# damien911224/ZeroShotVideoClassification

Measured on AMD Instinct MI355X. Metric: clips/sec (fwd+bwd+step) R(2+1)D-18 16x112x112 bs=22/GPU, higher is better.
Workload: dtype f32; 1 GPU; r2plus1d_18 training step (zero_grad+fwd+MSE+bwd+Adam), 22 clips/GPU 3x16x112x112, random-init, fp32 (BASELINE.json configs[1]); clips_per_gpu=22, global_batch=22, optimizer=Adam lr=1e-3 (torch.optim.Adam), parallelism=dp1, world_size=1, launcher=single process, input=resident

## Files before the change

### include/zsv_hip.h

```cpp
#ifndef ZSV_HIP_H
#define ZSV_HIP_H

#include <stddef.h>
#include <stdint.h>

#ifdef __cplusplus
extern "C" {
#endif

#define ZSV_OK 0
#define ZSV_E_BAD_SHAPE 1
#define ZSV_E_NULL 2
#define ZSV_E_WORKSPACE 3
#define ZSV_E_TOO_LARGE 4
#define ZSV_E_LAUNCH 5
#define ZSV_E_UNSUPPORTED 6

typedef struct zsv_conv_desc {
    int32_t N, Cin, Ti, Hi, Wi;
    int32_t Cout, To, Ho, Wo;
    int32_t kT, kH, kW;
    int32_t sT, sH, sW;
    int32_t pT, pH, pW;
} zsv_conv_desc;
// ... 21 lines not shown
                     void* workspace, size_t workspace_bytes, void* stream);
int32_t zsv_conv3d_dgrad_add_supported(const zsv_conv_desc* d);
int zsv_conv3d_dgrad_add(const zsv_conv_desc* d, const float* dy, const float* w, const float* add, float* dx,
                         void* workspace, size_t workspace_bytes, void* stream);
int32_t zsv_conv3d_dgrad_add_strided_supported(const zsv_conv_desc* d, int32_t st, int32_t sh, int32_t sw);
int zsv_conv3d_dgrad_add_strided(const zsv_conv_desc* d, const float* dy, const float* w, const float* sub, int32_t st, int32_t sh,
                                 int32_t sw, float* dx, void* workspace, size_t workspace_bytes, void* stream);
size_t zsv_conv3d_wgrad_workspace_bytes(const zsv_conv_desc* d);
int zsv_conv3d_wgrad(const zsv_conv_desc* d, const float* x, const float* dy, float* dw,
                     void* workspace, size_t workspace_bytes, void* stream);
size_t zsv_conv3d_wgrad_mask_bytes(const zsv_conv_desc* d);
int zsv_conv3d_wgrad_mask(const zsv_conv_desc* d, void* mask, void* stream);
int zsv_conv3d_wgrad_masked(const zsv_conv_desc* d, const float* x, const float* dy, float* dw, void* workspace,
                            size_t workspace_bytes, const void* mask, void* stream);

int zsv_bn_fwd_train_coeffs(const float* x, int32_t N, int32_t C, int32_t S, const float* gamma, const float* beta,
                            float* save_mean, float* save_invstd, float* running_mean, float* running_var, float momentum,
                            float eps, const float* conv_partials, int32_t stat_tiles, float* coef, int32_t coef_pitch,
                            void* workspace, size_t workspace_bytes, void* stream);
int32_t zsv_conv3d_pre_supported(const zsv_conv_desc* d);
int zsv_conv3d_fwd_pre(const zsv_conv_desc* d, const float* x, const float* pre_coef, int32_t coef_pitch, const float* w,
                       float* y, float* bn_partials, int32_t stat_tiles, void* workspace, size_t workspace_bytes,
                       void* stream);
int zsv_conv3d_wgrad_pre(const zsv_conv_desc* d, const float* x, const float* pre_coef, int32_t coef_pitch,
                         const float* dy, float* dw, void* workspace, size_t workspace_bytes, void* stream);
size_t zsv_channel_sum_workspace_bytes(int32_t N, int32_t C, int32_t S);
int zsv_channel_sum(const float* dy, int32_t N, int32_t C, int32_t S, float* db,
                    void* workspace, size_t workspace_bytes, void* stream);

size_t zsv_bn_workspace_bytes(int32_t N, int32_t C, int32_t S);
int zsv_bn_fwd_train(const float* x, int32_t N, int32_t C, int32_t S, const float* gamma,
                     const float* beta, const float* residual, int fuse_relu, float* y,
                     float* save_mean, float* save_invstd, float* running_mean,
                     float* running_var, float momentum, float eps, void* workspace,
                     size_t workspace_bytes, void* stream);
int zsv_bn_fwd_train_stats(const float* x, int32_t N, int32_t C, int32_t S, const float* gamma,
                           const float* beta, const float* residual, int fuse_relu, float* y,
                           float* save_mean, float* save_invstd, float* running_mean,
                           float* running_var, float momentum, float eps, const float* conv_partials,
                           int32_t stat_tiles, void* workspace, size_t workspace_bytes, void* stream);
int zsv_bn_fwd_eval(const float* x, int32_t N, int32_t C, int32_t S, const float* gamma,
                    const float* beta, const float* running_mean, const float* running_var,
                    const float* residual, int fuse_relu, float eps, float* y, void* workspace,
                    size_t workspace_bytes, void* stream);
int zsv_bn_bwd(const float* dy, const float* x, const float* y, int32_t N, int32_t C, int32_t S,
               const float* gamma, const float* beta, const float* save_mean, const float* save_invstd,
               int fuse_relu, float* dx, float* d_residual, float* dgamma, float* dbeta,
               void* workspace, size_t workspace_bytes, void* stream);
int zsv_bn_bwd_eval(const float* dy, const float* x, const float* y, int32_t N, int32_t C, int32_t S,
                    const float* gamma, const float* beta, const float* running_mean, const float* running_var, float eps,
                    int fuse_relu, float* dx, float* d_residual, float* dgamma, float* dbeta,
                    void* workspace, size_t workspace_bytes, void* stream);
int zsv_bn_eval_coeffs(int32_t C, const float* gamma, const float* beta, const float* running_mean, const float* running_var,
                       float eps, float* coef, int32_t coef_pitch, void* stream);

int zsv_relu_fwd(const float* x, float* y, int64_t n, void* stream);
int zsv_relu_bwd(const float* dy, const float* y, float* dx, int64_t n, void* stream);
int zsv_relu_bwd_bias(const float* dy, const float* y, float* dx, int32_t N, int32_t C, int32_t S, float* db,
                      void* workspace, size_t workspace_bytes, void* stream);
int zsv_add_relu_fwd(const float* a, const float* b, float* y, int64_t n, void* stream);

int zsv_meanpool_fwd(const float* x, int32_t N, int32_t C, int32_t S, float* y, void* stream);
int zsv_meanpool_bwd(const float* dy, int32_t N, int32_t C, int32_t S, float* dx, void* stream);
int zsv_maxpool3d_fwd(const float* x, int32_t N, int32_t C, int32_t Ti, int32_t Hi, int32_t Wi,
                      int32_t kT, int32_t kH, int32_t kW, int32_t pT, int32_t pH, int32_t pW,
                      int32_t To, int32_t Ho, int32_t Wo, float* y, int32_t* argmax, void* stream);
int zsv_maxpool3d_bwd(const float* dy, const int32_t* argmax, int32_t N, int32_t C, int32_t Ti,
                      int32_t Hi, int32_t Wi, int32_t kT, int32_t kH, int32_t kW, int32_t pT,
                      int32_t pH, int32_t pW, int32_t To, int32_t Ho, int32_t Wo, float* dx,
                      void* stream);

size_t zsv_linear_fwd_workspace_bytes(int32_t rows, int32_t in_features, int32_t out_features);
int zsv_linear_fwd(const float* x, const float* w, const float* bias, float* y, int32_t rows,
                   int32_t in_features, int32_t out_features, int fuse_relu, void* workspace,
                   size_t workspace_bytes, void* stream);
size_t zsv_linear_dgrad_workspace_bytes(int32_t rows, int32_t in_features, int32_t out_features);
int zsv_linear_dgrad(const float* dy, const float* w, float* dx, int32_t rows, int32_t in_features,
                     int32_t out_features, void* workspace, size_t workspace_bytes, void* stream);
size_t zsv_linear_wgrad_workspace_bytes(int32_t rows, int32_t in_features, int32_t out_features);
int zsv_linear_wgrad(const float* x, const float* dy, float* dw, int32_t rows,
                     int32_t in_features, int32_t out_features, void* workspace,
                     size_t workspace_bytes, void* stream);

size_t zsv_cosine_topk_workspace_bytes(int32_t rows, int32_t n_classes);
int zsv_cosine_topk(const float* embed, const float* class_embed, int32_t rows, int32_t dim, int32_t n_classes,
                    int32_t k, int32_t* out_index, double* out_dist, void* workspace, size_t workspace_bytes,
                    void* stream);

size_t zsv_split_accuracy_workspace_bytes(int32_t rows, int32_t n_classes);
int zsv_split_accuracy(const float* pred, const float* true_embed, const int64_t* labels, const float* class_embed,
                       int32_t rows, int32_t dim, int32_t n_classes, const int32_t* split_pos, int32_t n_tables,
                       int32_t* counts, int32_t* class_counts, void* workspace, size_t workspace_bytes, void* stream);

int zsv_adam_step(float* p, const float* g, float* exp_avg, float* exp_avg_sq, int64_t n,
                  float lr, float beta1, float beta2, float eps, int32_t step, void* stream);

int32_t zsv_bf16_channel_pitch(int32_t channels);
size_t zsv_conv3d_bf16_blob_bytes(const zsv_conv_desc* d);
int zsv_conv3d_bf16_pack(const zsv_conv_desc* d, const float* w, const float* scale, const float* shift,
                         void* blob, void* stream);
int zsv_conv3d_bf16_pack_dgrad(const zsv_conv_desc* d, const float* w_fwd, void* blob, void* stream);
int zsv_conv3d_bf16_fwd(const zsv_conv_desc* d, const void* x, const void* blob, const void* residual,
                        int fuse_relu, void* y, void* stream);
int32_t zsv_conv3d_bf16_stat_rows(const zsv_conv_desc* d);
int zsv_conv3d_bf16_fwd_stats(const zsv_conv_desc* d, const void* x, const void* blob, void* y, float* bn_partials,
                              int32_t rows_capacity, int32_t* rows, void* stream);
int zsv_clip_to_bf16(const float* x, int32_t N, int32_t C, int32_t T, int32_t H, int32_t W, int32_t padH,
                     int32_t padW, int32_t Hp, int32_t Wp, void* out, void* stream);
int zsv_maxpool3d_bf16(const void* x, int32_t N, int32_t C, int32_t Ti, int32_t Hi, int32_t Wi, int32_t kT, int32_t kH, int32_t kW,
                       int32_t pT, int32_t pH, int32_t pW, int32_t To, int32_t Ho, int32_t Wo, void* y, void* stream);
int zsv_meanpool_bf16(const void* x, int32_t N, int32_t S, int32_t C, float* out, void* stream);

int32_t zsv_fp8_channel_pitch(int32_t channels);
size_t zsv_conv3d_fp8_blob_bytes(const zsv_conv_desc* d);
int zsv_conv3d_fp8_pack(const zsv_conv_desc* d, const float* w, const float* scale, const float* shift, void* blob, void* stream);
int zsv_conv3d_fp8_fwd(const zsv_conv_desc* d, const void* x, const void* blob, const void* residual, int fuse_relu, void* y,
                       void* stream);
int zsv_meanpool_fp8(const void* x, int32_t N, int32_t S, int32_t C, float* out, void* stream);
int zsv_maxpool3d_fp8(const void* x, int32_t N, int32_t C, int32_t Ti, int32_t Hi, int32_t Wi, int32_t kT, int32_t kH, int32_t kW,
                      int32_t pT, int32_t pH, int32_t pW, int32_t To, int32_t Ho, int32_t Wo, void* y, void* stream);
int zsv_absmax_bf16(const void* x, int64_t count, float* amax, void* stream);

size_t zsv_bn_cl_workspace_bytes(int64_t R, int32_t C);
int zsv_bn_cl_fwd_train(const void* z, const void* residual, int64_t R, int32_t C, const float* gamma, const float* beta,
                        float* running_mean, float* running_var, float momentum, float eps, int fuse_relu, void* y,
                        float* save_mean, float* save_invstd, float* save_coef, void* workspace, size_t workspace_bytes, void* stream);
int zsv_bn_cl_fwd_train_stats(const void* z, const void* residual, int64_t R, int32_t C, const float* gamma, const float* beta,
                              float* running_mean, float* running_var, float momentum, float eps, int fuse_relu, void* y,
                              float* save_mean, float* save_invstd, float* save_coef, const float* conv_partials, int32_t conv_rows,
                              void* workspace, size_t workspace_bytes, void* stream);
int zsv_bn_cl_bwd(const void* dy, const void* y, const void* z, int64_t R, int32_t C, const float* gamma, const float* save_mean,
                  const float* save_invstd, const float* fwd_coef, int relu_mask, void* dz, void* g_out, float* dgamma, float* dbeta,
                  void* workspace, size_t workspace_bytes, void* stream);
int zsv_bn_cl_fwd_eval(const void* z, const void* residual, int64_t R, int32_t C, const float* gamma, const float* beta,
                       const float* running_mean, const float* running_var, float eps, int fuse_relu, void* y, float* coef,
                       void* stream);
int zsv_bn_cl_bwd_eval(const void* dy, const void* y, const void* z, int64_t R, int32_t C, const float* coef, int relu_mask, void* dz,
                       void* g_out, float* dgamma, float* dbeta, void* workspace, size_t workspace_bytes, void* stream);
size_t zsv_conv3d_bf16_wgrad_workspace_bytes(const zsv_conv_desc* d);
int zsv_conv3d_bf16_wgrad(const zsv_conv_desc* d, const void* x, const void* dz, float* dw, void* workspace, size_t workspace_bytes,
                          void* stream);
int zsv_maxpool3d_bf16_bwd(const void* dy, const void* x, int32_t N, int32_t C, int32_t Ti, int32_t Hi, int32_t Wi, int32_t kT, int32_t kH,
                           int32_t kW, int32_t pT, int32_t pH, int32_t pW, int32_t To, int32_t Ho, int32_t Wo, void* dx, void* stream);
int zsv_relu_bias_bwd_cl(const void* dy, const void* y, int64_t R, int32_t C, void* g_out, float* dbias, void* workspace,
                         size_t workspace_bytes, void* stream);
int zsv_cl_bf16_to_ncs_f32(const void* x, int32_t N, int32_t S, int32_t C, float* out, void* stream);
int zsv_ncs_f32_to_cl_bf16(const float* x, int32_t N, int32_t S, int32_t C, void* out, void* stream);
int zsv_meanpool_bf16_bwd(const float* dpooled, int32_t N, int32_t S, int32_t C, void* dx, void* stream);

int zsv_clip_transform(const uint8_t* frames_u8, int32_t N, int32_t T, int32_t Hin, int32_t Win,
                       int32_t Hres, int32_t Wres, float inv_scale, int32_t crop,
                       const int32_t* crop_flip_params_device, float* out, void* stream);
#define ZSV_CLIP_ROW 8
int zsv_clip_transform_batch(const int64_t* video_table_device, int32_t B, int32_t n_clips, int32_t T,
                             int32_t crop, float* out, void* stream);

int zsv_still_image_clips(const int64_t* image_table_device, const int32_t* frame_table_device, int32_t B,
                          int32_t n_clips, int32_t T, int32_t crop, int32_t max_side, float* out, void* stream);
int zsv_resample_coeffs(int32_t side, int32_t crop, int32_t* coeffs, int32_t* bounds, void* stream);

typedef struct zsv_adam_tensor {
    float* p;
    const float* g;
    float* exp_avg;
    float* exp_avg_sq;
    int64_t n;
// ... 114 lines not shown
```

### zeroshotvideoclassification_amd/_lib.py

```python
from __future__ import annotations

import ctypes
import os
import threading
from ctypes import POINTER, Structure, c_char_p, c_double, c_float, c_int, c_int32, c_int64, c_size_t, c_void_p

_HERE = os.path.dirname(os.path.abspath(__file__))
LIB_PATH = os.environ.get("ZSV_LIB_PATH") or os.path.join(_HERE, "libzsv_hip.so")


class ConvDesc(Structure):
    _fields_ = [(n, c_int32) for n in (
        "N", "Cin", "Ti", "Hi", "Wi", "Cout", "To", "Ho", "Wo",
        "kT", "kH", "kW", "sT", "sH", "sW", "pT", "pH", "pW")]


_P = c_void_p
SIGNATURES = {
    "zsv_status_string": (c_char_p, [c_int]),
    "zsv_version": (c_char_p, []),
    "zsv_reload_knobs": (c_int32, []),
    "zsv_conv3d_fwd_workspace_bytes": (c_size_t, [POINTER(ConvDesc)]),
    "zsv_conv3d_fwd": (c_int, [POINTER(ConvDesc), _P, _P, _P, _P, c_int, _P, c_size_t, _P]),
    "zsv_conv3d_fwd_stat_tiles": (c_int32, [POINTER(ConvDesc), _P]),
    "zsv_conv3d_fwd_stats": (c_int, [POINTER(ConvDesc), _P, _P, _P, _P, c_int, _P, c_int32, _P, c_size_t, _P]),
    "zsv_conv3d_fwd_add_supported": (c_int32, [POINTER(ConvDesc)]),
    "zsv_conv3d_fwd_add": (c_int, [POINTER(ConvDesc), _P, _P, _P, _P, _P, c_int, _P, c_size_t, _P]),
    "zsv_conv3d_fwd_full": (c_int, [POINTER(ConvDesc), _P, _P, _P, _P, _P, c_int, _P, c_int32, _P, c_size_t, _P]),
    "zsv_conv3d_dgrad_workspace_bytes": (c_size_t, [POINTER(ConvDesc)]),
    "zsv_conv3d_dgrad": (c_int, [POINTER(ConvDesc), _P, _P, _P, _P, c_size_t, _P]),
    "zsv_conv3d_dgrad_add_supported": (c_int32, [POINTER(ConvDesc)]),
    "zsv_conv3d_dgrad_add": (c_int, [POINTER(ConvDesc), _P, _P, _P, _P, _P, c_size_t, _P]),
    "zsv_conv3d_dgrad_add_strided_supported": (c_int32, [POINTER(ConvDesc), c_int32, c_int32, c_int32]),
    "zsv_conv3d_dgrad_add_strided": (c_int, [POINTER(ConvDesc), _P, _P, _P, c_int32, c_int32, c_int32, _P, _P, c_size_t, _P]),
    "zsv_conv3d_wgrad_workspace_bytes": (c_size_t, [POINTER(ConvDesc)]),
    "zsv_conv3d_wgrad": (c_int, [POINTER(ConvDesc), _P, _P, _P, _P, c_size_t, _P]),
    "zsv_conv3d_wgrad_mask_bytes": (c_size_t, [POINTER(ConvDesc)]),
    "zsv_conv3d_wgrad_mask": (c_int, [POINTER(ConvDesc), _P, _P]),
    "zsv_conv3d_wgrad_masked": (c_int, [POINTER(ConvDesc), _P, _P, _P, _P, c_size_t, _P, _P]),
    "zsv_bn_fwd_train_coeffs": (c_int, [_P, c_int32, c_int32, c_int32, _P, _P, _P, _P, _P, _P, c_float, c_float, _P, c_int32, _P,
                                        c_int32, _P, c_size_t, _P]),
    "zsv_conv3d_pre_supported": (c_int32, [POINTER(ConvDesc)]),
    "zsv_conv3d_fwd_pre": (c_int, [POINTER(ConvDesc), _P, _P, c_int32, _P, _P, _P, c_int32, _P, c_size_t, _P]),
    "zsv_conv3d_wgrad_pre": (c_int, [POINTER(ConvDesc), _P, _P, c_int32, _P, _P, _P, c_size_t, _P]),
    "zsv_channel_sum_workspace_bytes": (c_size_t, [c_int32, c_int32, c_int32]),
    "zsv_channel_sum": (c_int, [_P, c_int32, c_int32, c_int32, _P, _P, c_size_t, _P]),
    "zsv_bn_workspace_bytes": (c_size_t, [c_int32, c_int32, c_int32]),
    "zsv_bn_fwd_train": (c_int, [_P, c_int32, c_int32, c_int32, _P, _P, _P, c_int, _P, _P, _P, _P, _P,
                                 c_float, c_float, _P, c_size_t, _P]),
    "zsv_bn_fwd_train_stats": (c_int, [_P, c_int32, c_int32, c_int32, _P, _P, _P, c_int, _P, _P, _P, _P, _P,
                                       c_float, c_float, _P, c_int32, _P, c_size_t, _P]),
    "zsv_bn_fwd_eval": (c_int, [_P, c_int32, c_int32, c_int32, _P, _P, _P, _P, _P, c_int, c_float, _P, _P,
                                c_size_t, _P]),
    "zsv_bn_bwd": (c_int, [_P, _P, _P, c_int32, c_int32, c_int32, _P, _P, _P, _P, c_int, _P, _P, _P, _P, _P,
                           c_size_t, _P]),
    "zsv_bn_bwd_eval": (c_int, [_P, _P, _P, c_int32, c_int32, c_int32, _P, _P, _P, _P, c_float, c_int, _P, _P, _P, _P, _P,
                                c_size_t, _P]),
    "zsv_bn_eval_coeffs": (c_int, [c_int32, _P, _P, _P, _P, c_float, _P, c_int32, _P]),
    "zsv_relu_fwd": (c_int, [_P, _P, c_int64, _P]),
    "zsv_relu_bwd": (c_int, [_P, _P, _P, c_int64, _P]),
    "zsv_relu_bwd_bias": (c_int, [_P, _P, _P, c_int32, c_int32, c_int32, _P, _P, c_size_t, _P]),
    "zsv_add_relu_fwd": (c_int, [_P, _P, _P, c_int64, _P]),
    "zsv_meanpool_fwd": (c_int, [_P, c_int32, c_int32, c_int32, _P, _P]),
    "zsv_meanpool_bwd": (c_int, [_P, c_int32, c_int32, c_int32, _P, _P]),
    "zsv_maxpool3d_fwd": (c_int, [_P] + [c_int32] * 14 + [_P, _P, _P]),
    "zsv_maxpool3d_bwd": (c_int, [_P, _P] + [c_int32] * 14 + [_P, _P]),
    "zsv_linear_fwd_workspace_bytes": (c_size_t, [c_int32, c_int32, c_int32]),
    "zsv_linear_fwd": (c_int, [_P, _P, _P, _P, c_int32, c_int32, c_int32, c_int, _P, c_size_t, _P]),
    "zsv_linear_dgrad_workspace_bytes": (c_size_t, [c_int32, c_int32, c_int32]),
    "zsv_linear_dgrad": (c_int, [_P, _P, _P, c_int32, c_int32, c_int32, _P, c_size_t, _P]),
    "zsv_linear_wgrad_workspace_bytes": (c_size_t, [c_int32, c_int32, c_int32]),
    "zsv_linear_wgrad": (c_int, [_P, _P, _P, c_int32, c_int32, c_int32, _P, c_size_t, _P]),
    "zsv_bf16_channel_pitch": (c_int32, [c_int32]),
    "zsv_conv3d_bf16_blob_bytes": (c_size_t, [POINTER(ConvDesc)]),
    "zsv_conv3d_bf16_pack": (c_int, [POINTER(ConvDesc), _P, _P, _P, _P, _P]),
    "zsv_conv3d_bf16_pack_dgrad": (c_int, [POINTER(ConvDesc), _P, _P, _P]),
    "zsv_conv3d_bf16_fwd": (c_int, [POINTER(ConvDesc), _P, _P, _P, c_int, _P, _P]),
    "zsv_clip_to_bf16": (c_int, [_P] + [c_int32] * 9 + [_P, _P]),
    "zsv_maxpool3d_bf16": (c_int, [_P] + [c_int32] * 14 + [_P, _P]),
    "zsv_meanpool_bf16": (c_int, [_P, c_int32, c_int32, c_int32, _P, _P]),
    "zsv_fp8_channel_pitch": (c_int32, [c_int32]),
    "zsv_conv3d_fp8_blob_bytes": (c_size_t, [POINTER(ConvDesc)]),
    "zsv_conv3d_fp8_pack": (c_int, [POINTER(ConvDesc), _P, _P, _P, _P, _P]),
    "zsv_conv3d_fp8_fwd": (c_int, [POINTER(ConvDesc), _P, _P, _P, c_int, _P, _P]),
    "zsv_meanpool_fp8": (c_int, [_P, c_int32, c_int32, c_int32, _P, _P]),
    "zsv_maxpool3d_fp8": (c_int, [_P] + [c_int32] * 14 + [_P, _P]),
    "zsv_absmax_bf16": (c_int, [_P, c_int64, _P, _P]),
    "zsv_bn_cl_workspace_bytes": (c_size_t, [c_int64, c_int32]),
    "zsv_bn_cl_fwd_train": (c_int, [_P, _P, c_int64, c_int32, _P, _P, _P, _P, c_float, c_float, c_int, _P, _P, _P, _P, _P, c_size_t, _P]),
    "zsv_bn_cl_fwd_train_stats": (c_int, [_P, _P, c_int64, c_int32, _P, _P, _P, _P, c_float, c_float, c_int, _P, _P, _P, _P, _P, c_int32, _P,
                                          c_size_t, _P]),
    "zsv_conv3d_bf16_stat_rows": (c_int32, [POINTER(ConvDesc)]),
    "zsv_conv3d_bf16_fwd_stats": (c_int, [POINTER(ConvDesc), _P, _P, _P, _P, c_int32, _P, _P]),
    "zsv_bn_cl_bwd": (c_int, [_P, _P, _P, c_int64, c_int32, _P, _P, _P, _P, c_int, _P, _P, _P, _P, _P, c_size_t, _P]),
    "zsv_bn_cl_fwd_eval": (c_int, [_P, _P, c_int64, c_int32, _P, _P, _P, _P, c_float, c_int, _P, _P, _P]),
    "zsv_bn_cl_bwd_eval": (c_int, [_P, _P, _P, c_int64, c_int32, _P, c_int, _P, _P, _P, _P, _P, c_size_t, _P]),
    "zsv_conv3d_bf16_wgrad_workspace_bytes": (c_size_t, [POINTER(ConvDesc)]),
    "zsv_conv3d_bf16_wgrad": (c_int, [POINTER(ConvDesc), _P, _P, _P, _P, c_size_t, _P]),
    "zsv_maxpool3d_bf16_bwd": (c_int, [_P, _P] + [c_int32] * 14 + [_P, _P]),
    "zsv_relu_bias_bwd_cl": (c_int, [_P, _P, c_int64, c_int32, _P, _P, _P, c_size_t, _P]),
    "zsv_cl_bf16_to_ncs_f32": (c_int, [_P, c_int32, c_int32, c_int32, _P, _P]),
    "zsv_ncs_f32_to_cl_bf16": (c_int, [_P, c_int32, c_int32, c_int32, _P, _P]),
    "zsv_meanpool_bf16_bwd": (c_int, [_P, c_int32, c_int32, c_int32, _P, _P]),
    "zsv_clip_transform": (c_int, [_P, c_int32, c_int32, c_int32, c_int32, c_int32, c_int32, c_float, c_int32, _P, _P, _P]),
    "zsv_clip_transform_batch": (c_int, [_P, c_int32, c_int32, c_int32, c_int32, _P, _P]),
    "zsv_still_image_clips": (c_int, [_P, _P, c_int32, c_int32, c_int32, c_int32, c_int32, _P, _P]),
    "zsv_resample_coeffs": (c_int, [c_int32, c_int32, _P, _P, _P]),
    "zsv_cosine_topk_workspace_bytes": (c_size_t, [c_int32, c_int32]),
    "zsv_cosine_topk": (c_int, [_P, _P, c_int32, c_int32, c_int32, c_int32, _P, _P, _P, c_size_t, _P]),
    "zsv_split_accuracy_workspace_bytes": (c_size_t, [c_int32, c_int32]),
    "zsv_split_accuracy": (c_int, [_P, _P, _P, _P, c_int32, c_int32, c_int32, _P, c_int32, _P, _P, _P, c_size_t, _P]),
    "zsv_adam_multi": (c_int, [_P, c_int32, c_int64, c_float, c_float, c_float, c_float, c_int32, _P]),
    "zsv_grad_check_multi": (c_int, [_P, c_int32, c_int64, _P, _P]),
    "zsv_adam_multi_scaled": (c_int, [_P, c_int32, c_int64, c_float, c_float, c_float, c_float, _P, _P]),
    "zsv_scaler_update": (c_int, [_P, c_float, c_float, c_int32, _P]),
    "zsv_grad_norm_workspace_bytes": (c_size_t, [c_int64]),
    "zsv_grad_norm_multi": (c_int, [_P, c_int32, c_int64, c_int64, _P, c_size_t, _P, _P]),
    "zsv_grad_norm_finalize": (c_int, [_P, c_int64, c_float, _P, _P, _P]),
    "zsv_grad_unscale_multi": (c_int, [_P, c_int32, c_int64, _P, _P]),
    "zsv_adamw_multi": (c_int, [_P, c_int32, c_int64, c_double, c_float, c_float, c_float, c_double, c_int32, _P, c_int32, _P]),
    "zsv_adamw_multi_scaled": (c_int, [_P, c_int32, c_int64, c_double, c_float, c_float, c_float, c_double, c_int32, _P, _P,
                                       c_int32, _P]),
    "zsv_grad_accum_multi": (c_int, [_P, c_int32, c_int64, c_float, c_int32, _P]),
    "zsv_sgd_multi": (c_int, [_P, c_int32, c_int64, c_double, c_float, c_float, c_int32, c_double, c_int32, _P, _P, c_int32, c_int32,
                              _P, _P, c_float, _P]),
    "zsv_adam_multi_avg": (c_int, [_P, c_int32, c_int64, c_float, c_float, c_float, c_float, c_int32, _P, _P, c_float, _P]),
    "zsv_adam_multi_scaled_avg": (c_int, [_P, c_int32, c_int64, c_float, c_float, c_float, c_float, _P, _P, _P, c_float, _P]),
    "zsv_adamw_multi_avg": (c_int, [_P, c_int32, c_int64, c_double, c_float, c_float, c_float, c_double, c_int32, _P, c_int32,
                                    _P, _P, c_float, _P]),
    "zsv_adamw_multi_scaled_avg": (c_int, [_P, c_int32, c_int64, c_double, c_float, c_float, c_float, c_double, c_int32, _P, _P,
                                           c_int32, _P, _P, c_float, _P]),
    "zsv_avg_multi": (c_int, [_P, c_int32, c_int64, _P, c_float, _P, _P]),
    "zsv_avg_advance": (c_int, [_P, _P, _P]),
    "zsv_swap_multi": (c_int, [_P, c_int32, c_int64, _P]),
    "zsv_adam_step": (c_int, [_P, _P, _P, _P, c_int64, c_float, c_float, c_float, c_float, c_int32, _P]),
    "zsv_conv3d_panel_query": (c_int, [POINTER(ConvDesc), c_int32, c_int32, POINTER(c_size_t)]),
    "zsv_conv3d_panel_job": (c_int, [POINTER(ConvDesc), c_int32, c_int32, _P, _P, c_size_t, _P]),
    "zsv_pack_multi": (c_int, [_P, c_int32, c_int64, _P]),
    "zsv_conv3d_fwd_full_panel": (c_int, [POINTER(ConvDesc), _P, _P, _P, _P, _P, c_int, _P, c_int32, _P, c_size_t, _P, _P, c_size_t]),
    "zsv_conv3d_fwd_pre_panel": (c_int, [POINTER(ConvDesc), _P, _P, c_int32, _P, _P, _P, c_int32, _P, c_size_t, _P, _P, c_size_t]),
    "zsv_conv3d_dgrad_add_panel": (c_int, [POINTER(ConvDesc), _P, _P, _P, _P, _P, c_size_t, _P, _P, c_size_t]),
    "zsv_conv3d_dgrad_add_strided_panel": (c_int, [POINTER(ConvDesc), _P, _P, _P, c_int32, c_int32, c_int32, _P, _P, c_size_t, _P, _P,
                                                   c_size_t]),
}


class PackJob(Structure):
    _fields_ = [("kind", c_int32), ("reserved", c_int32), ("total", c_int64), ("first_block", c_int64), ("w", c_void_p),
                ("out", c_void_p), ("l", c_int64 * 2), ("i", c_int32 * 20)]

_lock = threading.Lock()
# ... 86 lines not shown
```

### zeroshotvideoclassification_amd/csrc/knobs.h

```cpp
#pragma once

#define ZSV_KNOB_LIST(X) \
    X(NO_FUSED_STATS) \
    X(NO_BN_FUSION) \
    X(BF16_NO_SAME) \
    X(BF16_NO_TSAME) \
    X(BF16_NO_SAME64) \
    X(BF16_NO_SAME9) \
    X(BF16_SAME9_MIN_CHUNKS) \
    X(WINOT_NO_T32) \
    X(BF16_GROUP_OUTER) \
    X(BF16_NO_WGRAD) \
    X(BF16_NO_WGRAD_GATHER) \
    X(BF16_WGRAD_WGS) \
    X(NO_DGRAD_S2) \
    X(NO_DGRAD_S2T) \
    X(DGRAD_S2_BN) \
    X(DGRAD_S2_KS) \
    X(NO_DOWN_FUSION) \
    X(DGRAD_S2_NO_X4) \
    X(CONV_CFG) \
    X(NO_SPLITK) \
    X(TAP_KS) \
    X(SPLITK_THRESH) \
    X(NO_CFG5) \
    X(NO_TAP) \
    X(NO_LDS_EPILOGUE) \
    X(WGRAD_CFG) \
    X(WGRAD_BN) \
    X(WGRAD_WGS) \
    X(WGRAD_NO_TWOTAP) \
    X(NO_WGRAD_DMA) \
    X(WGRAD_DMA_TM) \
    X(WGRAD_DMA_TN) \
    X(WGRAD_DMA_SLICES) \
    X(WGRAD_LINEAR_WALK) \
    X(NO_STEM_WGRAD) \
    X(STEM_WGRAD_WGS) \
    X(WGRAD_TRING_RESIDENT) \
    X(WGRAD_TRING_SLICES) \
    X(NO_WGRAD_TRING) \
    X(NO_WGRAD_TWINO) \
    X(WGRAD_WINO_SLICES) \
    X(NO_WINO) \
    X(NO_WGRAD_WINO) \
    X(NO_WGRAD_WINO4) \
    X(WINO_MIN_TILES) \
    X(WINO_NO_SPLITK) \
    X(NO_WINOT) \
    X(WINOT_MIN_TILES) \
    X(BN_NT_MB) \
    X(BN_NO_MASKED_G) \
    X(WINOT_MAX_WASTE) \
    X(NO_WINO_FWD) \
    X(WINO_NO_F43) \
    X(WINOT_NO_F43) \
    X(WINO_NO_X4) \
    X(NO_SLAB_SUM_ROWS) \
    X(SPLITK_REDUCE_SCALAR) \
    X(NO_PACK_TILED) \
    X(NO_T2_DENSE) \
    X(WINO_NO_VW) \
    X(WINO_VW_MIN_WGS) \
    X(WINOT_GENERIC_EPILOGUE) \
    X(WINO_GENERIC_EPILOGUE)

namespace zsv {
enum KnobId {
#define ZSV_KNOB_ENUM(name) K_##name,
    ZSV_KNOB_LIST(ZSV_KNOB_ENUM)
#undef ZSV_KNOB_ENUM
    K_COUNT
};
extern const char* volatile g_knobs[K_COUNT];
}

#define ZSV_KNOB(name) (::zsv::g_knobs[::zsv::K_##name])
```

### zeroshotvideoclassification_amd/network.py

```python
from __future__ import annotations

import torch
import torch.nn.functional as F
from torch import nn

from . import ops
from . import resnet as models
from .layers import Conv3d, Linear, MaxPool3d, ReLU


def get_network(opt):
    name = opt.network
    if "r3d" in name:
        factory = models.r3d_18
    elif "2plus1d" in name:
        factory = models.r2plus1d_18
    elif "c3d" in name:
        return C3D(fixconvs=opt.fixconvs, nopretrained=opt.nopretrained)
    else:
        raise Exception("Network {} not available!".format(name))
    return Model(factory, fixconvs=opt.fixconvs, nopretrained=opt.nopretrained)


def _freeze(module: nn.Module) -> None:
    for p in module.parameters():
        p.requires_grad = False


class MLP(nn.Module):

    def __init__(self, input_dim, hidden_dim, output_dim, num_layers, last_activate=False):
        super().__init__()
        self.num_layers = num_layers
        self.last_activate = last_activate
        widths = [input_dim] + [hidden_dim] * (num_layers - 1) + [output_dim]
        self.layers = nn.ModuleList(Linear(a, b) for a, b in zip(widths[:-1], widths[1:]))

    def forward(self, x):
        last = self.num_layers - 1
        for i, layer in enumerate(self.layers):
            x = layer(x, relu=(i < last))
        return x


class Model(nn.Module):

    def __init__(self, network, fixconvs=False, nopretrained=False):
        super().__init__()
        self.model = network(pretrained=nopretrained)
        if fixconvs:
            _freeze(self.model)
        self.d_model = 256
        self.num_sentences = 1
        self.t_pos_embeds = nn.Embedding(self.num_sentences, 512)
        self.special_tokens = nn.Embedding(1, self.d_model)
        self.feature2input_proj = nn.Linear(512, self.d_model)
        self.encoder = nn.TransformerEncoder(
            nn.TransformerEncoderLayer(d_model=self.d_model, dim_feedforward=self.d_model * 4, nhead=8, dropout=0.1,
                                       activation="gelu"),
            num_layers=6, enable_nested_tensor=False)
        self.output2emb_proj = MLP(512, 512, 300, 2)
        self.reset_parameters()

    def reset_parameters(self):
        nn.init.normal_(self.t_pos_embeds.weight)
        nn.init.xavier_uniform_(self.special_tokens.weight)

    def forward(self, x):
        bs, nc, ch, t, h, w = x.shape
        from . import amp
        if amp.is_autocast_enabled() and x.is_cuda:
            from . import resnet
            if isinstance(self.model, resnet.VideoResNet):
                if self.training:
                    pooled = amp.trunk_features(self.model, x.reshape(bs * nc, ch, t, h, w))
                    return F.normalize(self.output2emb_proj(pooled)), None
                if not torch.is_grad_enabled():
                    from .inference import engine_for
                    return engine_for(self, torch.bfloat16)(x)
        _, feats = self.model(x.reshape(bs * nc, ch, t, h, w))
        pooled = ops.mean_pool(feats)
        emb = F.normalize(self.output2emb_proj(pooled))
        return emb, None


class ResNet18(nn.Module):

    def __init__(self, network, fixconvs=False, nopretrained=True):
        super().__init__()
        self.model = network(pretrained=nopretrained)
        if fixconvs:
            _freeze(self.model)
        self.regressor = Linear(self.model.fc.in_features, 300)
        self.dropout = nn.Dropout(p=0.05)

    def forward(self, x):
        bs, nc, ch, t, h, w = x.shape
        pooled, _ = self.model(x.reshape(bs * nc, ch, t, h, w))
        pooled = pooled.reshape(bs, nc, -1).mean(1)
        return F.normalize(self.regressor(self.dropout(pooled)))


class C3D(nn.Module):

    def __init__(self, fixconvs=False, nopretrained=True):
        super().__init__()
        three = (3, 3, 3)
        one = (1, 1, 1)
        self.conv1 = Conv3d(3, 64, kernel_size=three, padding=one)
        self.pool1 = MaxPool3d(kernel_size=(1, 2, 2), stride=(1, 2, 2))
        self.conv2 = Conv3d(64, 128, kernel_size=three, padding=one)
        self.pool2 = MaxPool3d(kernel_size=(2, 2, 2), stride=(2, 2, 2))
        self.conv3a = Conv3d(128, 256, kernel_size=three, padding=one)
        self.conv3b = Conv3d(256, 256, kernel_size=three, padding=one)
        self.pool3 = MaxPool3d(kernel_size=(2, 2, 2), stride=(2, 2, 2))
        self.conv4a = Conv3d(256, 512, kernel_size=three, padding=one)
        self.conv4b = Conv3d(512, 512, kernel_size=three, padding=one)
        self.pool4 = MaxPool3d(kernel_size=(2, 2, 2), stride=(2, 2, 2))
        self.conv5a = Conv3d(512, 512, kernel_size=three, padding=one)
        self.conv5b = Conv3d(512, 512, kernel_size=three, padding=one)
        self.pool5 = MaxPool3d(kernel_size=(2, 2, 2), stride=(2, 2, 2), padding=(0, 1, 1))
        self.fc6 = Linear(8192, 4096)
        self.fc7 = Linear(4096, 4096)
        self.fc8 = Linear(4096, 487)
        self.dropout = nn.Dropout(p=0.10)
        self.relu = ReLU()
        self.softmax = nn.Softmax()
        if nopretrained:
            self.load_state_dict(torch.load("./assets/c3d.pickle"))
        self.regressor = Linear(4096, 300)
        if fixconvs:
            for m in (self.conv1, self.conv2, self.conv3a, self.conv3b, self.conv4a, self.conv4b, self.conv5a,
                      self.conv5b, self.fc6):
                _freeze(m)

    def forward(self, x):
        bs, nc, ch, t, h, w = x.shape
        from . import amp
        if amp.is_autocast_enabled() and x.is_cuda:
            if not torch.is_grad_enabled() and not self.training:
                from .inference import engine_for
                return engine_for(self, torch.bfloat16)(x)
            if torch.is_grad_enabled():
                a = amp.c3d_features(self, x.reshape(bs * nc, ch, t, h, w))
                a = self.fc6(a, relu=True)
                a = self.dropout(a)
                a = a.reshape(bs, nc, -1).mean(1).reshape(bs, -1)
                return F.normalize(self.regressor(a), dim=-1)
        a = x.reshape(bs * nc, ch, t, h, w)
        a = self.pool1(self.conv1(a, relu=True))
        a = self.pool2(self.conv2(a, relu=True))
        a = self.pool3(self.conv3b(self.conv3a(a, relu=True), relu=True))
        a = self.pool4(self.conv4b(self.conv4a(a, relu=True), relu=True))
        a = self.pool5(self.conv5b(self.conv5a(a, relu=True), relu=True))
        a = self.fc6(a.reshape(-1, 8192), relu=True)
        a = self.dropout(a)
        a = a.reshape(bs, nc, -1).mean(1).reshape(bs, -1)
        return F.normalize(self.regressor(a), dim=-1)
```

### zeroshotvideoclassification_amd/ops.py

```python
from __future__ import annotations

import os
import threading

from ctypes import byref, c_size_t, c_void_p
from typing import Optional, Sequence, Tuple

import torch
from torch.autograd import Function
from torch.autograd.function import once_differentiable

from . import _lib
from ._lib import ConvDesc


def _triple(v) -> Tuple[int, int, int]:
    if isinstance(v, int):
        return (v, v, v)
    v = tuple(int(a) for a in v)
    if len(v) == 1:
        return (v[0],) * 3
    if len(v) != 3:
        raise ValueError(f"expected an int or 3 ints, got {v}")
    return v
# ... 998 lines not shown
        dx = torch.empty(geom[:5], dtype=torch.float32, device=dy.device)
        with torch.cuda.device(dy.device):
            _lib.check(_lib.load().zsv_maxpool3d_bwd(dy.data_ptr(), arg.data_ptr(), *geom, dx.data_ptr(), _stream()),
                       "zsv_maxpool3d_bwd")
        return dx, None, None


def max_pool3d(x, kernel_size, stride=None, padding=0):
    k = _triple(kernel_size)
    s = k if stride is None else _triple(stride)
    if s != k:
        raise RuntimeError("max_pool3d: only kernel_size == stride is implemented (all the reference uses)")
    return _MaxPool3d.apply(x, k, _triple(padding))


class _Linear(Function):

    @staticmethod
    def forward(ctx, x, weight, bias, relu):
        _require(x, weight, bias)
        if x.dim() != 2:
            raise RuntimeError("linear expects a (rows, in_features) input")
        x, weight = x.contiguous(), weight.contiguous()
        rows, fin = int(x.shape[0]), int(x.shape[1])
        fout = int(weight.shape[0])
        if int(weight.shape[1]) != fin:
            raise RuntimeError("linear: in_features mismatch")
        y = torch.empty((rows, fout), dtype=torch.float32, device=x.device)
        lib = _lib.load()
        nbytes = lib.zsv_linear_fwd_workspace_bytes(rows, fin, fout)
        ws = _workspace(nbytes, x.device)
        with torch.cuda.device(x.device):
            _lib.check(lib.zsv_linear_fwd(x.data_ptr(), weight.data_ptr(), _ptr(bias), y.data_ptr(), rows, fin,
                                          fout, 1 if relu else 0, _ptr(ws), nbytes, _stream()), "zsv_linear_fwd")
        ctx.dims = (rows, fin, fout)
        ctx.relu = bool(relu)
        ctx.has_bias = bias is not None
        ctx.save_for_backward(x, weight, y if relu else None)
        return y

    @staticmethod
    @once_differentiable
    def backward(ctx, dy):
        x, weight, y = ctx.saved_tensors
        rows, fin, fout = ctx.dims
        lib = _lib.load()
        dy = dy.contiguous()
        dx = dw = db = None
        with torch.cuda.device(dy.device):
            if ctx.relu:
                g = torch.empty_like(dy)
                if ctx.has_bias and ctx.needs_input_grad[2]:
                    n_, c_ = int(dy.shape[0]), int(dy.shape[1])
                    s_ = dy.numel() // (n_ * c_)
                    db = torch.empty(c_, dtype=torch.float32, device=dy.device)
                    nb = lib.zsv_channel_sum_workspace_bytes(n_, c_, s_)
                    wsb = _workspace(nb, dy.device)
                    _lib.check(lib.zsv_relu_bwd_bias(dy.data_ptr(), y.data_ptr(), g.data_ptr(), n_, c_, s_, db.data_ptr(),
                                                     _ptr(wsb), nb, _stream()), "zsv_relu_bwd_bias")
                else:
                    _lib.check(lib.zsv_relu_bwd(dy.data_ptr(), y.data_ptr(), g.data_ptr(), g.numel(), _stream()), "zsv_relu_bwd")
                dy = g
            if ctx.needs_input_grad[0]:
                dx = torch.empty_like(x)
                nbytes = lib.zsv_linear_dgrad_workspace_bytes(rows, fin, fout)
                ws = _workspace(nbytes, dy.device)
                _lib.check(lib.zsv_linear_dgrad(dy.data_ptr(), weight.data_ptr(), dx.data_ptr(), rows, fin, fout,
                                                _ptr(ws), nbytes, _stream()), "zsv_linear_dgrad")
            if ctx.needs_input_grad[1]:
                dw = torch.empty_like(weight)
                nbytes = lib.zsv_linear_wgrad_workspace_bytes(rows, fin, fout)
                ws = _workspace(nbytes, dy.device)
                _lib.check(lib.zsv_linear_wgrad(x.data_ptr(), dy.data_ptr(), dw.data_ptr(), rows, fin, fout, _ptr(ws),
                                                nbytes, _stream()), "zsv_linear_wgrad")
            if ctx.has_bias and ctx.needs_input_grad[2] and db is None:
                db = channel_sum(dy)
        return dx, dw, db, None


def linear(x, weight, bias=None, relu=False):
    return _Linear.apply(x, weight, bias, bool(relu))


def adam_step_(p: torch.Tensor, g: torch.Tensor, exp_avg: torch.Tensor, exp_avg_sq: torch.Tensor, step: int,
               lr: float, betas=(0.9, 0.999), eps: float = 1e-8) -> None:
    _require(p, g, exp_avg, exp_avg_sq)
    for t in (p, g, exp_avg, exp_avg_sq):
        if not t.is_contiguous() or t.numel() != p.numel():
            raise RuntimeError("adam_step_: flat contiguous buffers of equal size expected")
    with torch.cuda.device(p.device):
        _lib.check(_lib.load().zsv_adam_step(p.data_ptr(), g.data_ptr(), exp_avg.data_ptr(), exp_avg_sq.data_ptr(),
                                             p.numel(), float(lr), float(betas[0]), float(betas[1]), float(eps),
                                             int(step), _stream()), "zsv_adam_step")
```

Baseline: 578.8 clips/s.

## Fuse mean-pool, two-layer MLP head and L2 normalize into single HIP kernels

Adds a fused forward kernel that does spatial mean pooling, Linear+ReLU, Linear and L2 normalization per row in one block. A matching fused backward kernel computes the input gradient and all weight and bias gradients. This replaces several small launches (mean pool, linear, normalize and their backward ops) in the model head, cutting launch overhead and intermediate traffic. The kernels accumulate in fp64 and each handles a whole row per block, so they may run slower than tuned GEMMs if the head dimensions are large.

```diff
diff --git a/include/zsv_hip.h b/include/zsv_hip.h
--- a/include/zsv_hip.h
+++ b/include/zsv_hip.h
@@ -127,6 +127,14 @@
                      int32_t in_features, int32_t out_features, void* workspace,
                      size_t workspace_bytes, void* stream);
 
+int32_t zsv_head_supported(int32_t R, int32_t C, int32_t S, int32_t H, int32_t O);
+int zsv_head_fwd(const float* feats, int32_t R, int32_t C, int32_t S, const float* w1, const float* b1, int32_t H,
+                 const float* w2, const float* b2, int32_t O, float eps, float* e, float* p, float* h, float* norm,
+                 void* stream);
+int zsv_head_bwd(const float* de, const float* e, const float* p, const float* h, const float* norm, const float* w1,
+                 const float* w2, int32_t R, int32_t C, int32_t S, int32_t H, int32_t O, float eps, float* dfeats,
+                 float* dw1, float* db1, float* dw2, float* db2, void* stream);
+
 size_t zsv_cosine_topk_workspace_bytes(int32_t rows, int32_t n_classes);
 int zsv_cosine_topk(const float* embed, const float* class_embed, int32_t rows, int32_t dim, int32_t n_classes,
                     int32_t k, int32_t* out_index, double* out_dist, void* workspace, size_t workspace_bytes,
diff --git a/zeroshotvideoclassification_amd/_lib.py b/zeroshotvideoclassification_amd/_lib.py
--- a/zeroshotvideoclassification_amd/_lib.py
+++ b/zeroshotvideoclassification_amd/_lib.py
@@ -67,6 +67,9 @@
     "zsv_maxpool3d_bwd": (c_int, [_P, _P] + [c_int32] * 14 + [_P, _P]),
     "zsv_linear_fwd_workspace_bytes": (c_size_t, [c_int32, c_int32, c_int32]),
     "zsv_linear_fwd": (c_int, [_P, _P, _P, _P, c_int32, c_int32, c_int32, c_int, _P, c_size_t, _P]),
+    "zsv_head_supported": (c_int32, [c_int32] * 5),
+    "zsv_head_fwd": (c_int, [_P, c_int32, c_int32, c_int32, _P, _P, c_int32, _P, _P, c_int32, c_float, _P, _P, _P, _P, _P]),
+    "zsv_head_bwd": (c_int, [_P] * 7 + [c_int32] * 5 + [c_float] + [_P] * 6),
     "zsv_linear_dgrad_workspace_bytes": (c_size_t, [c_int32, c_int32, c_int32]),
     "zsv_linear_dgrad": (c_int, [_P, _P, _P, c_int32, c_int32, c_int32, _P, c_size_t, _P]),
     "zsv_linear_wgrad_workspace_bytes": (c_size_t, [c_int32, c_int32, c_int32]),
diff --git a/zeroshotvideoclassification_amd/csrc/head.hip b/zeroshotvideoclassification_amd/csrc/head.hip
--- /dev/null
+++ b/zeroshotvideoclassification_amd/csrc/head.hip
@@ -0,0 +1,298 @@
+#include <hip/hip_runtime.h>
+#include <stdint.h>
+#include "zsv_hip.h"
+#include "zsv_common.h"
+#include "knobs.h"
+
+namespace zsv {
+
+constexpr int HEAD_THREADS = 1024;
+constexpr int HEAD_WAVES = HEAD_THREADS / 64;
+constexpr int HEAD_JB = 8;
+constexpr int HEAD_U = 8;
+constexpr size_t HEAD_LDS_MAX = 96 * 1024;
+
+static inline int pad4(int n) { return (n + 3) & ~3; }
+__device__ __forceinline__ int dpad4(int n) { return (n + 3) & ~3; }
+
+template <bool VEC>
+__device__ __forceinline__ void rows_matvec(const float* __restrict__ W, const float* __restrict__ bias, const float* v, float* out,
+                                            float* __restrict__ keep, int J, int I, bool relu) {
+    const int lane = threadIdx.x & 63, wave = threadIdx.x >> 6;
+    for (int j0 = wave * HEAD_U; j0 < J; j0 += HEAD_WAVES * HEAD_U) {
+        double acc[HEAD_U];
+#pragma unroll
+        for (int u = 0; u < HEAD_U; ++u) acc[u] = 0.0;
+        if (VEC) {
+            for (int i = 4 * lane; i < I; i += 256) {
+                const float4 a = *reinterpret_cast<const float4*>(v + i);
+#pragma unroll
+                for (int u = 0; u < HEAD_U; ++u) {
+                    const int j = min(j0 + u, J - 1);
+                    const float4 w = *reinterpret_cast<const float4*>(W + (size_t)j * I + i);
+                    acc[u] = fma((double)w.x, (double)a.x, acc[u]);
+                    acc[u] = fma((double)w.y, (double)a.y, acc[u]);
+                    acc[u] = fma((double)w.z, (double)a.z, acc[u]);
+                    acc[u] = fma((double)w.w, (double)a.w, acc[u]);
+                }
+            }
+        } else {
+            for (int i = lane; i < I; i += 64) {
+                const double a = (double)v[i];
+#pragma unroll
+                for (int u = 0; u < HEAD_U; ++u) {
+                    const int j = min(j0 + u, J - 1);
+                    acc[u] = fma((double)W[(size_t)j * I + i], a, acc[u]);
+                }
+            }
+        }
+#pragma unroll
+        for (int u = 0; u < HEAD_U; ++u) acc[u] = wave_sum(acc[u]);
+        if (lane == 0) {
+#pragma unroll
+            for (int u = 0; u < HEAD_U; ++u) {
+                const int j = j0 + u;
+                if (j < J) {
+                    float a = (float)(acc[u] + (bias ? (double)bias[j] : 0.0));
+                    if (relu) a = fmaxf(a, 0.f);
+                    out[j] = a;
+                    if (keep) keep[j] = a;
+                }
+            }
+        }
+    }
+}
+
+__global__ __launch_bounds__(HEAD_THREADS) void head_fwd_kernel(const float* __restrict__ feats, int C, int S,
+                                                                const float* __restrict__ w1, const float* __restrict__ b1, int H,
+                                                                const float* __restrict__ w2, const float* __restrict__ b2, int O,
+                                                                float eps, float* __restrict__ e, float* __restrict__ p_keep,
+                                                                float* __restrict__ h_keep, float* __restrict__ nrm_keep, int vec1,
+                                                                int vec2) {
+    extern __shared__ __attribute__((aligned(16))) unsigned char head_lds[];
+    float* p = reinterpret_cast<float*>(head_lds);
+    float* h = p + dpad4(C);
+    float* y = h + dpad4(H);
+    __shared__ float s_norm;
+    const int r = blockIdx.x, lane = threadIdx.x & 63, wave = threadIdx.x >> 6;
+    const float* f = feats + (size_t)r * C * S;
+    for (int c0 = wave * 4; c0 < C; c0 += HEAD_WAVES * 4) {
+        double a[4] = {0.0, 0.0, 0.0, 0.0};
+        for (int s = lane; s < S; s += 64) {
+#pragma unroll
+            for (int u = 0; u < 4; ++u) a[u] += (double)f[(size_t)min(c0 + u, C - 1) * S + s];
+        }
+#pragma unroll
+        for (int u = 0; u < 4; ++u) a[u] = wave_sum(a[u]);
+        if (lane == 0) {
+#pragma unroll
+            for (int u = 0; u < 4; ++u) {
+                if (c0 + u < C) {
+                    const float m = (float)(a[u] / (double)S);
+                    p[c0 + u] = m;
+                    p_keep[(size_t)r * C + c0 + u] = m;
+                }
+            }
+        }
+    }
+    __syncthreads();
+    if (vec1) rows_matvec<true>(w1, b1, p, h, h_keep + (size_t)r * H, H, C, true);
+    else rows_matvec<false>(w1, b1, p, h, h_keep + (size_t)r * H, H, C, true);
+    __syncthreads();
+    if (vec2) rows_matvec<true>(w2, b2, h, y, nullptr, O, H, false);
+    else rows_matvec<false>(w2, b2, h, y, nullptr, O, H, false);
+    __syncthreads();
+    if (wave == 0) {
+        double q = 0.0;
+        for (int o = lane; o < O; o += 64) q = fma((double)y[o], (double)y[o], q);
+        q = wave_sum(q);
+        if (lane == 0) {
+            s_norm = (float)sqrt(q);
+            nrm_keep[r] = s_norm;
+        }
+    }
+    __syncthreads();
+    const float denom = fmaxf(s_norm, eps);
+    for (int o = threadIdx.x; o < O; o += HEAD_THREADS) e[(size_t)r * O + o] = y[o] / denom;
+}
+
+__device__ __forceinline__ void wave_row_dy(const float* __restrict__ e_r, const float* __restrict__ de_r, float nrm, float eps, int O,
+                                            float* dst, int lane) {
+    double d = 0.0;
+    for (int o = lane; o < O; o += 64) d = fma((double)e_r[o], (double)de_r[o], d);
+    d = wave_sum(d);
+    const double denom = (double)fmaxf(nrm, eps);
+    const bool live = nrm >= eps;
+    for (int o = lane; o < O; o += 64) dst[o] = (float)((live ? fma(-(double)e_r[o], d, (double)de_r[o]) : (double)de_r[o]) / denom);
+}
+
+__device__ __forceinline__ void cols_matvec(const float* __restrict__ M, int I, int J, const float* v, double* part, float* out,
+                                            const float* __restrict__ mask, double div) {
+    const int lane = threadIdx.x & 63, wave = threadIdx.x >> 6;
+    const int chunk = (I + HEAD_WAVES - 1) / HEAD_WAVES;
+    const int i0 = min(I, wave * chunk), i1 = min(I, i0 + chunk);
+    for (int jb = 0; jb < J; jb += 256) {
+        double a[4] = {0.0, 0.0, 0.0, 0.0};
+        for (int i = i0; i < i1; ++i) {
+            const double x = (double)v[i];
+#pragma unroll
+            for (int u = 0; u < 4; ++u) {
+                const int j = min(jb + 64 * u + lane, J - 1);
+                a[u] = fma(x, (double)M[(size_t)i * J + j], a[u]);
+            }
+        }
+#pragma unroll
+        for (int u = 0; u < 4; ++u) {
+            const int j = jb + 64 * u + lane;
+            if (j < J) part[(size_t)wave * J + j] = a[u];
+        }
+    }
+    __syncthreads();
+    for (int j = threadIdx.x; j < J; j += HEAD_THREADS) {
+        double s = 0.0;
+        for (int w = 0; w < HEAD_WAVES; ++w) s += part[(size_t)w * J + j];
+        if (mask && !(mask[j] > 0.f)) s = 0.0;
+        out[j] = (float)(s / div);
+    }
+    __syncthreads();
+}
+
+__global__ __launch_bounds__(HEAD_THREADS) void head_bwd_kernel(const float* __restrict__ de, const float* __restrict__ e,
+                                                                const float* __restrict__ p, const float* __restrict__ h,
+                                                                const float* __restrict__ nrm, const float* __restrict__ w1,
+                                                                const float* __restrict__ w2, int R, int C, int S, int H, int O,
+                                                                float eps, int row_blocks, float* __restrict__ dfeats,
+                                                                float* __restrict__ dw1, float* __restrict__ db1,
+                                                                float* __restrict__ dw2, float* __restrict__ db2) {
+    extern __shared__ __attribute__((aligned(16))) unsigned char head_lds[];
+    const int tid = threadIdx.x, lane = tid & 63, wave = tid >> 6;
+    if ((int)blockIdx.x < row_blocks) {
+        const int r = blockIdx.x;
+        double* part = reinterpret_cast<double*>(head_lds);
+        float* dy = reinterpret_cast<float*>(part + (size_t)HEAD_WAVES * max(H, C));
+        float* dpre = dy + dpad4(O);
+        float* dp = dpre + dpad4(H);
+        if (wave == 0) wave_row_dy(e + (size_t)r * O, de + (size_t)r * O, nrm[r], eps, O, dy, lane);
+        __syncthreads();
+        cols_matvec(w2, O, H, dy, part, dpre, h + (size_t)r * H, 1.0);
+        cols_matvec(w1, H, C, dpre, part, dp, nullptr, (double)S);
+        float* g = dfeats + (size_t)r * C * S;
+        const int total = C * S;
+        for (int i = tid; i < total; i += HEAD_THREADS) g[i] = dp[i / S];
+        return;
+    }
+    const int jblk = (int)blockIdx.x - row_blocks;
+    const int j0 = jblk * HEAD_JB, jn = min(HEAD_JB, H - j0);
+    const int RJ = R * HEAD_JB;
+    double* part = reinterpret_cast<double*>(head_lds);
+    float* dy = reinterpret_cast<float*>(part + max(RJ, HEAD_THREADS));
+    float* dpre = dy + dpad4(R * O);
+    for (int r = wave; r < R; r += HEAD_WAVES) wave_row_dy(e + (size_t)r * O, de + (size_t)r * O, nrm[r], eps, O, dy + (size_t)r * O, lane);
+    __syncthreads();
+    const int nparts = RJ >= HEAD_THREADS ? 1 : min(HEAD_WAVES, HEAD_THREADS / RJ);
+    const int ochunk = (O + nparts - 1) / nparts;
+    for (int idx = tid; idx < nparts * RJ; idx += HEAD_THREADS) {
+        const int pi = idx / RJ, q = idx - pi * RJ, r = q / HEAD_JB, jj = q - r * HEAD_JB;
+        const int o0 = min(O, pi * ochunk), o1 = min(O, o0 + ochunk);
+        double a = 0.0;
+        if (jj < jn) {
+            for (int o = o0; o < o1; ++o) a = fma((double)dy[(size_t)r * O + o], (double)w2[(size_t)o * H + j0 + jj], a);
+        }
+        part[idx] = a;
+    }
+    __syncthreads();
+    for (int q = tid; q < RJ; q += HEAD_THREADS) {
+        const int r = q / HEAD_JB, jj = q - r * HEAD_JB;
+        double s = 0.0;
+        for (int pi = 0; pi < nparts; ++pi) s += part[pi * RJ + q];
+        dpre[q] = (jj < jn && h[(size_t)r * H + j0 + jj] > 0.f) ? (float)s : 0.f;
+    }
+    __syncthreads();
+    if (dw1) {
+        for (int idx = tid; idx < jn * C; idx += HEAD_THREADS) {
+            const int jj = idx / C, c = idx - jj * C;
+            double a = 0.0;
+            for (int r = 0; r < R; ++r) a = fma((double)dpre[r * HEAD_JB + jj], (double)p[(size_t)r * C + c], a);
+            dw1[(size_t)(j0 + jj) * C + c] = (float)a;
+        }
+    }
+    if (db1 && tid < jn) {
+        double a = 0.0;
+        for (int r = 0; r < R; ++r) a += (double)dpre[r * HEAD_JB + tid];
+        db1[j0 + tid] = (float)a;
+    }
+    if (dw2) {
+        for (int idx = tid; idx < O * jn; idx += HEAD_THREADS) {
+            const int o = idx / jn, jj = idx - o * jn;
+            double a = 0.0;
+            for (int r = 0; r < R; ++r) a = fma((double)dy[(size_t)r * O + o], (double)h[(size_t)r * H + j0 + jj], a);
+            dw2[(size_t)o * H + j0 + jj] = (float)a;
+        }
+    }
+    if (db2 && jblk == 0) {
+        for (int o = tid; o < O; o += HEAD_THREADS) {
+            double a = 0.0;
+            for (int r = 0; r < R; ++r) a += (double)dy[(size_t)r * O + o];
+            db2[o] = (float)a;
+        }
+    }
+}
+
+static inline size_t head_fwd_lds(int C, int H, int O) { return (size_t)(pad4(C) + pad4(H) + pad4(O)) * sizeof(float); }
+static inline size_t head_bwd_row_lds(int C, int H, int O) {
+    return (size_t)HEAD_WAVES * (H > C ? H : C) * sizeof(double) + (size_t)(pad4(O) + pad4(H) + pad4(C)) * sizeof(float);
+}
+static inline size_t head_bwd_hid_lds(int R, int O) {
+    const long rj = (long)R * HEAD_JB;
+    return (size_t)(rj > HEAD_THREADS ? rj : HEAD_THREADS) * sizeof(double) + (size_t)(pad4(R * O) + pad4((int)rj)) * sizeof(float);
+}
+static int head_check(int R, int C, int S, int H, int O) {
+    if (R <= 0 || C <= 0 || S <= 0 || H <= 0 || O <= 0) return ZSV_E_BAD_SHAPE;
+    if ((double)R * C * S >= 2147483647.0 || (double)H * C >= 2147483647.0 || (double)O * H >= 2147483647.0) return ZSV_E_TOO_LARGE;
+    if ((double)R * O >= 1e6 || (double)R * HEAD_JB >= 1e6) return ZSV_E_UNSUPPORTED;
+    if (head_fwd_lds(C, H, O) > HEAD_LDS_MAX || head_bwd_row_lds(C, H, O) > HEAD_LDS_MAX || head_bwd_hid_lds(R, O) > HEAD_LDS_MAX)
+        return ZSV_E_UNSUPPORTED;
+    return ZSV_OK;
+}
+
+}
+
+using namespace zsv;
+
+extern "C" int32_t zsv_head_supported(int32_t R, int32_t C, int32_t S, int32_t H, int32_t O) {
+    return (!ZSV_KNOB(NO_FUSED_HEAD) && head_check(R, C, S, H, O) == ZSV_OK) ? 1 : 0;
+}
+
+extern "C" int zsv_head_fwd(const float* feats, int32_t R, int32_t C, int32_t S, const float* w1, const float* b1, int32_t H,
+                            const float* w2, const float* b2, int32_t O, float eps, float* e, float* p, float* h, float* norm,
+                            void* stream) {
+    int st = head_check(R, C, S, H, O);
+    if (st) return st;
+    if (!feats || !w1 || !w2 || !e || !p || !h || !norm) return ZSV_E_NULL;
+    static const hipError_t attr = hipFuncSetAttribute((const void*)head_fwd_kernel, hipFuncAttributeMaxDynamicSharedMemorySize,
+                                                       (int)HEAD_LDS_MAX);
+    if (attr != hipSuccess) return ZSV_E_LAUNCH;
+    const int vec1 = (C % 4 == 0) && ((reinterpret_cast<uintptr_t>(w1) & 15) == 0);
+    const int vec2 = (H % 4 == 0) && ((reinterpret_cast<uintptr_t>(w2) & 15) == 0);
+    hipLaunchKernelGGL(head_fwd_kernel, dim3((unsigned)R), dim3(HEAD_THREADS), head_fwd_lds(C, H, O), (hipStream_t)stream, feats, C, S,
+                       w1, b1, H, w2, b2, O, eps, e, p, h, norm, vec1, vec2);
+    return launch_status();
+}
+
+extern "C" int zsv_head_bwd(const float* de, const float* e, const float* p, const float* h, const float* norm, const float* w1,
+                            const float* w2, int32_t R, int32_t C, int32_t S, int32_t H, int32_t O, float eps, float* dfeats,
+                            float* dw1, float* db1, float* dw2, float* db2, void* stream) {
+    int st = head_check(R, C, S, H, O);
+    if (st) return st;
+    if (!de || !e || !p || !h || !norm || !w1 || !w2) return ZSV_E_NULL;
+    static const hipError_t attr = hipFuncSetAttribute((const void*)head_bwd_kernel, hipFuncAttributeMaxDynamicSharedMemorySize,
+                                                       (int)HEAD_LDS_MAX);
+    if (attr != hipSuccess) return ZSV_E_LAUNCH;
+    const int row_blocks = dfeats ? R : 0;
+    const int hid_blocks = (dw1 || db1 || dw2 || db2) ? (H + HEAD_JB - 1) / HEAD_JB : 0;
+    if (row_blocks + hid_blocks == 0) return ZSV_OK;
+    const size_t a = row_blocks ? head_bwd_row_lds(C, H, O) : 0, b = hid_blocks ? head_bwd_hid_lds(R, O) : 0;
+    hipLaunchKernelGGL(head_bwd_kernel, dim3((unsigned)(row_blocks + hid_blocks)), dim3(HEAD_THREADS), a > b ? a : b,
+                       (hipStream_t)stream, de, e, p, h, norm, w1, w2, R, C, S, H, O, eps, row_blocks, dfeats, dw1, db1, dw2, db2);
+    return launch_status();
+}
diff --git a/zeroshotvideoclassification_amd/csrc/knobs.h b/zeroshotvideoclassification_amd/csrc/knobs.h
--- a/zeroshotvideoclassification_amd/csrc/knobs.h
+++ b/zeroshotvideoclassification_amd/csrc/knobs.h
@@ -51,6 +51,7 @@
     X(WINOT_MIN_TILES) \
     X(BN_NT_MB) \
     X(BN_NO_MASKED_G) \
+    X(NO_FUSED_HEAD) \
     X(WINOT_MAX_WASTE) \
     X(NO_WINO_FWD) \
     X(WINO_NO_F43) \
diff --git a/zeroshotvideoclassification_amd/network.py b/zeroshotvideoclassification_amd/network.py
--- a/zeroshotvideoclassification_amd/network.py
+++ b/zeroshotvideoclassification_amd/network.py
@@ -66,6 +66,24 @@
         nn.init.normal_(self.t_pos_embeds.weight)
         nn.init.xavier_uniform_(self.special_tokens.weight)
 
+    def _fused_head_applies(self, feats) -> bool:
+        mlp = self.output2emb_proj
+        if type(mlp) is not MLP or mlp.num_layers != 2 or mlp.last_activate or len(mlp.layers) != 2:
+            return False
+        a, b = mlp.layers
+        params = (a.weight, a.bias, b.weight, b.bias)
+        if type(a) is not Linear or type(b) is not Linear or any(p is None for p in params):
+            return False
+        if models._has_hooks(mlp, mlp.layers, a, b):
+            return False
+        if not (feats.is_cuda and feats.dtype == torch.float32 and feats.dim() >= 2 and feats.numel() > 0):
+            return False
+        if any(p.dtype != torch.float32 or p.device != feats.device for p in params):
+            return False
+        if len({bool(p.requires_grad) for p in params}) != 1:
+            return False
+        return ops.head_supported(feats, a.weight, b.weight)
+
     def forward(self, x):
         bs, nc, ch, t, h, w = x.shape
         from . import amp
@@ -79,6 +97,9 @@
                     from .inference import engine_for
                     return engine_for(self, torch.bfloat16)(x)
         _, feats = self.model(x.reshape(bs * nc, ch, t, h, w))
+        if self._fused_head_applies(feats):
+            a, b = self.output2emb_proj.layers
+            return ops.fused_head(feats, a.weight, a.bias, b.weight, b.bias), None
         pooled = ops.mean_pool(feats)
         emb = F.normalize(self.output2emb_proj(pooled))
         return emb, None
diff --git a/zeroshotvideoclassification_amd/ops.py b/zeroshotvideoclassification_amd/ops.py
--- a/zeroshotvideoclassification_amd/ops.py
+++ b/zeroshotvideoclassification_amd/ops.py
@@ -1104,6 +1104,64 @@
     return _Linear.apply(x, weight, bias, bool(relu))
 
 
+NORMALIZE_EPS = 1e-12
+
+
+class _Head(Function):
+
+    @staticmethod
+    def forward(ctx, feats, w1, b1, w2, b2):
+        _require(feats, w1, b1, w2, b2)
+        feats, w1, b1, w2, b2 = (t.contiguous() for t in (feats, w1, b1, w2, b2))
+        r, c = int(feats.shape[0]), int(feats.shape[1])
+        s = feats.numel() // (r * c)
+        h, o = int(w1.shape[0]), int(w2.shape[0])
+        if tuple(w1.shape) != (h, c) or tuple(w2.shape) != (o, h) or tuple(b1.shape) != (h,) or tuple(b2.shape) != (o,):
+            raise RuntimeError("fused head: parameter shapes do not form Linear(C, H) -> Linear(H, O)")
+        dev = feats.device
+        e = torch.empty((r, o), dtype=torch.float32, device=dev)
+        p = torch.empty((r, c), dtype=torch.float32, device=dev)
+        hid = torch.empty((r, h), dtype=torch.float32, device=dev)
+        norm = torch.empty((r,), dtype=torch.float32, device=dev)
+        with torch.cuda.device(dev):
+            _lib.check(_lib.load().zsv_head_fwd(feats.data_ptr(), r, c, s, w1.data_ptr(), b1.data_ptr(), h, w2.data_ptr(),
+                                                b2.data_ptr(), o, NORMALIZE_EPS, e.data_ptr(), p.data_ptr(), hid.data_ptr(),
+                                                norm.data_ptr(), _stream()), "zsv_head_fwd")
+        ctx.dims = (r, c, s, h, o)
+        ctx.feats_shape = tuple(feats.shape)
+        ctx.save_for_backward(e, p, hid, norm, w1, w2)
+        return e
+
+    @staticmethod
+    @once_differentiable
+    def backward(ctx, de):
+        e, p, hid, norm, w1, w2 = ctx.saved_tensors
+        r, c, s, h, o = ctx.dims
+        de = de.contiguous()
+        dev = de.device
+        need = ctx.needs_input_grad
+        dfeats = torch.empty(ctx.feats_shape, dtype=torch.float32, device=dev) if need[0] else None
+        dw1 = torch.empty_like(w1) if need[1] else None
+        db1 = torch.empty((h,), dtype=torch.float32, device=dev) if need[2] else None
+        dw2 = torch.empty_like(w2) if need[3] else None
+        db2 = torch.empty((o,), dtype=torch.float32, device=dev) if need[4] else None
+        with torch.cuda.device(dev):
+            _lib.check(_lib.load().zsv_head_bwd(de.data_ptr(), e.data_ptr(), p.data_ptr(), hid.data_ptr(), norm.data_ptr(),
+                                                w1.data_ptr(), w2.data_ptr(), r, c, s, h, o, NORMALIZE_EPS, _ptr(dfeats), _ptr(dw1),
+                                                _ptr(db1), _ptr(dw2), _ptr(db2), _stream()), "zsv_head_bwd")
+        return dfeats, dw1, db1, dw2, db2
+
+
+def head_supported(feats, w1, w2) -> bool:
+    r, c = int(feats.shape[0]), int(feats.shape[1])
+    s = feats.numel() // max(1, r * c)
+    return bool(_lib.load().zsv_head_supported(r, c, s, int(w1.shape[0]), int(w2.shape[0])))
+
+
+def fused_head(feats, w1, b1, w2, b2):
+    return _Head.apply(feats, w1, b1, w2, b2)
+
+
 def adam_step_(p: torch.Tensor, g: torch.Tensor, exp_avg: torch.Tensor, exp_avg_sq: torch.Tensor, step: int,
                lr: float, betas=(0.9, 0.999), eps: float = 1e-8) -> None:
     _require(p, g, exp_avg, exp_avg_sq)
```

Result: no change. 580.7 clips/s, median of 6 (+0.3%).
